# gift-surg/NSoL

Hardware: AMD Instinct MI355X
Metric: primal-dual iters/sec on 512^3 fp32 TV-L2 (higher is better)
Workload: dtype f32

## Files before the change

include/nsol_hip.h:

```cpp
#ifndef NSOL_HIP_H
#define NSOL_HIP_H

#include <stdint.h>

#ifdef __cplusplus
extern "C" {
#endif

#define NSOL_HIP_ABI_VERSION 1
#define NSOL_EINVAL (-1)

#define NSOL_MODE_CONSTANT 0
#define NSOL_MODE_WRAP 1
#define NSOL_MODE_NEAREST 2
#define NSOL_MODE_REFLECT 3
#define NSOL_MODE_MIRROR 4

#define NSOL_PD_REG_TV 0
#define NSOL_PD_REG_HUBER 1
#define NSOL_PD_DATA_L2 0
#define NSOL_PD_DATA_L1 2
#define NSOL_PD_REG_ISOTROPIC 4
#define NSOL_PD_DATA_WEIGHTED 8
#define NSOL_PD_RUN_X_MAY_SWAP 0x100
// ... 255 lines not shown
                            int64_t nx, double wx, double wy, double wz, int k,
                            const double *sigma_k, const double *hden_k,
                            const double *tau_k, const double *tl_k,
                            const double *theta_k, int flags, void *stream);
int nsol_pd_fusedk_tuned(int elem_size, int k, int64_t nz, int64_t ny, int64_t nx);
int nsol_pd_fusedk_launches(int k);
int nsol_pd_fusedk_tail2(int elem_size, int64_t nz, int64_t ny, int64_t nx);
int nsol_pd_fusedk_plan(int elem_size, int k, int64_t nz, int64_t ny, int64_t nx,
                        int *waves, int *ntx, int64_t *zchunk);
int nsol_pd_shift_launches(void);
int nsol_pd_shift_min_iters(int elem_size, int ndim, int64_t nz, int64_t ny, int64_t nx,
                            int flags, int64_t pitch);
int nsol_pd_fusedk_plan_form(int elem_size, int k, int64_t nz, int64_t ny, int64_t nx,
                             int form, int *waves, int *ntx, int64_t *zchunk);
int nsol_pd_run_parts(int iterations, int min_iters, int *lead, int *launches);
int64_t nsol_pd_persist_ws_bytes(int elem_size, int ndim, int64_t nz, int64_t ny,
                                 int64_t nx, int iterations);
int nsol_pd_persist_run_f32(float *xbar, float *x, const float *bt, float *p, int ndim,
                            int64_t nz, int64_t ny, int64_t nx, double wx, double wy,
                            double wz, double lambda, const double *sigma_host,
                            const double *tau_host, const double *theta_host,
                            int iterations, int p_is_zero, double gamma_huber, int flags,
                            void *ws, int64_t ws_bytes, unsigned int *err_word,
                            void *stream);
int nsol_pd_persist_run_f64(double *xbar, double *x, const double *bt, double *p, int ndim,
                            int64_t nz, int64_t ny, int64_t nx, double wx, double wy,
                            double wz, double lambda, const double *sigma_host,
                            const double *tau_host, const double *theta_host,
                            int iterations, int p_is_zero, double gamma_huber, int flags,
                            void *ws, int64_t ws_bytes, unsigned int *err_word,
// ... 578 lines not shown
```

nsol_amd/_lib.py:

```python
import ctypes
import os
import re

HERE = os.path.dirname(os.path.abspath(__file__))
LIB_PATH = os.path.join(HERE, "csrc", "libnsol_hip.so")
HEADER = os.path.join(HERE, "..", "include", "nsol_hip.h")

_lib = None

c_i64 = ctypes.c_int64
c_int = ctypes.c_int
c_dbl = ctypes.c_double
c_ptr = ctypes.c_void_p

_CTYPE = {"int": c_int, "int64_t": c_i64, "double": c_dbl}


class NsolHipError(RuntimeError):
    pass


def declared_symbols(header=HEADER):
    text = open(header).read()
    text = re.sub(r"/\*.*?\*/", "", text, flags=re.S)
# ... 64 lines not shown
    return lib


def check(rc, what):
    if rc != 0:
        if rc == -1:
            raise ValueError("%s: invalid argument" % what)
        raise NsolHipError("%s failed with hipError_t %d" % (what, rc))


PARAM_DEFAULTS = {
    "pd_zchunk": 0, "pd_ry": 0, "pd_two_pass": 0, "pd_xcd_map": 1, "pd_rag": 1,
    "max_grid_blocks": 2048, "stencil_slabs": 1, "stencil_blocks": 65536,
    "pd2_zchunk": 0, "pd2_enable": 1, "pd2_variant": 0, "pd2_xcd_map": 1,
    "pdk_enable": 1, "pdk_kmax": 3, "pdk_nw": 0, "pdk_zchunk": 0, "pdk_ntx": 0,
    "pdk_xcd_map": 1, "pdk_verbose": 0, "pdk_autotune": 1, "pdk_pf2": -1,
    "pdk_split": -1, "pdk_tail2": 1, "pdk_min_kvox": 1024, "pdk_tune_min_mvox": 16,
    "pdk_shift": -1, "pdk_shift_min_iters": 30,
    "pdp_max_spin": 1 << 21, "pdp_mute_tile": -1,
    "corr_ra": 8, "corr_xv": 1, "corr_blur3_lxb": 16, "corr_blur3_zchunk": 0, "corr_blur3_dma": 1, "corr_blur3_dma_rag": 1, "lb_gram_dma": 1, "lb_gram_mfma": 1, "sort_walk_by_key": 1,
}
_touched = set()


def reset_params():
    for name in sorted(_touched):
        set_param(name, PARAM_DEFAULTS[name])
    _touched.clear()


def set_param(name, value):
# ... 19 lines not shown
```

nsol_amd/csrc/nsol_pd_common.hpp:

```cpp
#pragma once

#include "nsol_common.hpp"

namespace nsol {

template <typename T, int V>
struct Pack {
  typedef T type __attribute__((ext_vector_type(V)));
};

template <typename T, int V>
__device__ __forceinline__ void ldv(const T *p, T (&v)[V]) {
  if constexpr (V == 1) {
    v[0] = *p;
  } else {
    typedef typename Pack<T, V>::type P;
    const P t = *reinterpret_cast<const P *>(p);
#pragma unroll
    for (int k = 0; k < V; ++k) v[k] = t[k];
  }
}

template <typename T, int V>
__device__ __forceinline__ void stv(T *p, const T (&v)[V]) {
// ... 114 lines not shown
                   const double *hden, const double *tau, const double *tl,
                   const double *theta, int flags, void *stream, int64_t pitch);

template <typename T>
int pd_shift3_min_iters(const T *x, const T *x_alt, const T *bt, const T *p0, const T *p1,
                        int ndim, int64_t nz, int64_t ny, int64_t nx, int flags,
                        int64_t pitch, int iterations);
template <typename T>
int pd_shift3_donation(int64_t nz, int64_t ny, int64_t nx);
template <typename T>
int pd_shift3_iter(const T *x_in, T *x_out, const T *bt, const T *p_in, T *p_out, int ndim,
                   int64_t nz, int64_t ny, int64_t nx, double wx, double wy, double wz,
                   const double *sigma, const double *hden, const double *tau,
                   const double *tl, const double *theta, int flags, void *stream);

template <bool L1, typename T>
__device__ __forceinline__ T prox_data_s(T u, T bt, T tl, T one_plus_tl) {
  if constexpr (L1) return prox_ell1(u, bt, tl);
  else return prox_ell2(u, bt, tl, one_plus_tl);
}

}
```

nsol_amd/csrc/nsol_pdk.hip:

```cpp
#include <stdio.h>
#include <string.h>

#include <algorithm>
#include <atomic>
#include <deque>
#include <map>
#include <mutex>
#include <tuple>
#include <type_traits>
#include <vector>

#include "nsol_common.hpp"
#include "nsol_pd_common.hpp"

using namespace nsol;

#ifndef PDK_LH
#define PDK_LH 1
#endif
#ifndef PDK_ABLATE
#define PDK_ABLATE 0
#endif
#ifndef PDK_PRIO
#define PDK_PRIO 0
#endif
#ifndef PDK_LOAD_AUX
#define PDK_LOAD_AUX 0
#endif

namespace nsol_pdk {

template <typename T, int K>
struct StageScalars {
  T sigma[K], hden[K], tau[K], tl[K], optl[K], theta[K];
  int has_p;
};

std::atomic<int> g_launches[2];
std::atomic<int> g_shift_launches;

struct Tiling {
  int lxb;
  int rows;
  int xv;
// ... 111 lines not shown
};

template <typename T, int V>
struct PlaneLoads {
  T xn[V], xv[V], btn[V], pxo[V], pyo[V], pzo[V], xdown[V], xup[V], pyup[V];
  T xright, xleft, pxleft;
};

template <typename T, int VEC, int NW, int K, int WPE, bool HUBER, bool L1, bool PF2,
          bool UNIT, bool RAG>
__global__ __launch_bounds__(NW * 64, WPE) void k_pd_fusedk(
    const T *__restrict__ xbar_in, T *__restrict__ xbar_out,
    const T *__restrict__ x_in, T *__restrict__ x_out,
    const T *__restrict__ bt, const T *__restrict__ p_in,
    T *__restrict__ p_out, Geom<T> G, StageScalars<T, K> S, Tiling Q, int zchunk,
    int slab) {
  constexpr int NT = NW * 64;
  constexpr int H = K - 1;
  constexpr int HX = ((H + VEC - 1) / VEC) * VEC;
  constexpr int LN = LdsShape<NT, K>::N;
  constexpr bool LH = PDK_LH && K == 3 && NW == 12 && !PF2 && sizeof(T) == 4 && !RAG;
  constexpr int NB = LH ? 1 : 2;
  __shared__ __attribute__((aligned(16))) T s_xb[NB][K - 1][LN * VEC];
  __shared__ __attribute__((aligned(16))) T s_py[NB][K - 1][LN * VEC];
  __shared__ T s_px[NB][K - 1][LN];
  __shared__ __attribute__((aligned(16))) T s_xb0[LH ? LN * VEC : VEC];
  __shared__ __attribute__((aligned(16))) T s_py0[LH ? LN * VEC : VEC];
  __shared__ T s_px0[LH ? LN : 1];

  const int tid = threadIdx.x;
  const int lane = tid & 63;
  const int ntiles = Q.ntx * Q.nty;
  int tile, zc;
  if (slab > 0) {
    const int xcd = blockIdx.x & 7;
    const int j = blockIdx.x >> 3;
    tile = xcd * slab + j % slab;
    zc = j / slab;
    if (tile >= ntiles) return;
  } else {
    tile = blockIdx.x % ntiles;
    zc = blockIdx.x / ntiles;
  }
  const int tx = tile % Q.ntx;
  const int ty = tile / Q.ntx;

  const int lxb = Q.lxb;
  constexpr int HL = HX / VEC;
  int row, lx;
  bool lone = false;
  if (Q.split) {
    const int inner = lxb - 2 * HL;
    const int main = Q.rows * inner;
    if (tid < main) {
      row = tid / inner;
      lx = HL + (tid - row * inner);
      lone = (lx == HL) || (lx == HL + inner - 1);
    } else {
// ... 479 lines not shown
  if constexpr (PF2) {
    for (; s + 1 <= s_hi; s += 2) {
      step(std::true_type{}, s, LA, LB, CA, CB);
      step(std::true_type{}, s + 1, LB, LA, CB, CA);
    }
    if (s <= s_hi) {
      step(std::true_type{}, s, LA, LB, CA, CB);
      CA = CB;
      ++s;
    }
  } else {
    for (; s <= s_hi; ++s) step(std::true_type{}, s, LA, LA, CA, CA);
  }
  for (; s <= s_last; ++s)
    step(std::false_type{}, s, LA, LA, CA, CA);
}

template <typename T>
struct ShiftScalars {
  T sigma[4], hden[4];
  T tau[3], tl[3], optl[3], theta[3];
};

template <typename T, int V>
struct ShiftLoads {
  T xv[V], btn[V], pxo[V], pyo[V], pzo[V], pyup[V];
  T pxleft;
};

template <typename T, int VEC, int NW, int WPE, bool HUBER, bool L1, bool PF2, bool UNIT>
__global__ __launch_bounds__(NW * 64, WPE) void k_pd_shift3(
    const T *__restrict__ x_in, T *__restrict__ x_out, const T *__restrict__ bt,
    const T *__restrict__ p_in, T *__restrict__ p_out, Geom<T> G, ShiftScalars<T> S,
    Tiling Q, int zchunk, int slab) {
  constexpr int K = 3;
  constexpr int NT = NW * 64;
  constexpr int HA = 2, HB = 3;
  constexpr int HX = ((K + VEC - 1) / VEC) * VEC;
  static_assert(HX >= K, "the x halo must hold the three voxels the right-hand cone needs");
  constexpr int LN = LdsShape<NT, K>::N;
  __shared__ __attribute__((aligned(16))) T s_xb[2][K][LN * VEC];
  __shared__ __attribute__((aligned(16))) T s_py[2][LN * VEC];
  __shared__ T s_px[2][LN];

  const int tid = threadIdx.x;
  const int lane = tid & 63;
  const int ntiles = Q.ntx * Q.nty;
  int tile, zc;
  if (slab > 0) {
    const int xcd = blockIdx.x & 7;
    const int j = blockIdx.x >> 3;
    tile = xcd * slab + j % slab;
    zc = j / slab;
    if (tile >= ntiles) return;
  } else {
    tile = blockIdx.x % ntiles;
    zc = blockIdx.x / ntiles;
  }
  const int tx = tile % Q.ntx;
  const int ty = tile / Q.ntx;

  const int lxb = Q.lxb;
  constexpr int HL = HX / VEC;
  int row, lx;
  bool lone = false;
  if (Q.split) {
    const int inner = lxb - 2 * HL;
    const int main = Q.rows * inner;
    if (tid < main) {
      row = tid / inner;
      lx = HL + (tid - row * inner);
      lone = (lx == HL) || (lx == HL + inner - 1);
    } else {
// ... 294 lines not shown
  if constexpr (PF2) {
    for (; s + 1 <= s_hi; s += 2) {
      step(std::true_type{}, s, LA, LB, CA, CB);
      step(std::true_type{}, s + 1, LB, LA, CB, CA);
    }
    if (s <= s_hi) {
      step(std::true_type{}, s, LA, LB, CA, CB);
      CA = CB;
      ++s;
    }
  } else {
    for (; s <= s_hi; ++s) step(std::true_type{}, s, LA, LA, CA, CA);
  }
  for (; s <= s_last; ++s)
    step(std::false_type{}, s, LA, LA, CA, CA);
}

struct Tuning {
  int enable = 1;
  int kmax = 3;
  int nw = 0;
  int zchunk = 0;
  int ntx = 0;
  int xcd_map = 1;
  int verbose = 0;
  int autotune = 1;
  int tune_min_mvox = 16;
  int pf2 = -1;
  int tail2 = 1;
  int min_kvox = 1024;
};
Tuning g_tunek;

int g_split = -1;

struct Config {
  int nw = 0;
  int pf2 = 0;
  Tiling q{};
  int64_t zchunk = 0;
  double cost = 0.0;
};

inline bool make_tiling(int64_t nx, int64_t ny, int nt, int vec, int h, int hx,
                        int lxm, int ntx, Tiling *out, int64_t xv_fixed = 0, int lost = -1) {
  if (lost < 0) lost = 2 * h;
  Tiling q;
  if (ntx == 1) {
    q.xv = 0;
    q.lxb = (int)((nx + vec - 1) / vec);
  } else {
    int64_t xv = xv_fixed > 0 ? xv_fixed : (nx + ntx - 1) / ntx;
    xv = (xv + vec - 1) / vec * vec;
    if (xv * (ntx - 1) >= nx) return false;
    q.xv = (int)xv;
    q.lxb = (int)(xv / vec) + 2 * (hx / vec);
  }
  if (q.lxb < 1 || q.lxb > lxm) return false;
  q.rows = nt / q.lxb;
  if (q.rows - lost < 1) return false;
  q.ntx = ntx;
  q.nty = (int)((ny + (q.rows - lost) - 1) / (q.rows - lost));
  q.split = (ntx > 1 && (q.xv / vec) % 32 == 0 && g_split != 0) ? 1 : 0;
  *out = q;
  return true;
}

inline double pick_zchunk(int64_t nz, int64_t tiles, int extra, int64_t max_chunk,
                          int64_t *chunk_out) {
  const double slots = (double)cu_count();
  double best = -1.0;
  int64_t best_chunk = nz < max_chunk ? nz : max_chunk;
  for (int64_t nzc = 1; nzc <= nz; ++nzc) {
    const int64_t chunk = (nz + nzc - 1) / nzc;
    if (chunk < 8 && nzc > 1) break;
    if (chunk > max_chunk) continue;
    if ((nz + chunk - 1) / chunk != nzc) continue;
    const double blocks = (double)tiles * nzc;
    const double rounds = (double)(int64_t)((blocks + slots - 1) / slots);
    const double fill = blocks / (rounds * slots);
// ... 3 lines not shown
  *chunk_out = best_chunk;
  return best > 0.0 ? best : 1.0;
}

inline double model_cost(const Tiling &q, int64_t nx, int64_t ny, int64_t nz,
                         int vec, int esize, int h, int hx, double zeff, bool shift = false) {
  double lines = 0.0;
  for (int tx = 0; tx < q.ntx; ++tx) {
    int64_t lo = q.xv ? (int64_t)tx * q.xv - hx : 0;
    int64_t hi = lo + (int64_t)q.lxb * vec;
    if (lo < 0) lo = 0;
    if (hi > nx) hi = nx;
    if (hi <= lo) continue;
    lines += (double)((hi * esize - 1) / 128 - (lo * esize) / 128 + 1);
  }
  double rows = 0.0;
  const int64_t tyv = q.rows - (shift ? 2 * h + 1 : 2 * h);
  for (int ty = 0; ty < q.nty; ++ty) {
    int64_t lo = (int64_t)ty * tyv - h, hi = lo + q.rows;
    if (lo < 0) lo = 0;
    if (hi > ny) hi = ny;
    if (hi > lo) rows += (double)(hi - lo);
  }
  const double reads = lines * 128.0 * rows * (double)nz * (shift ? 5.0 : 6.0);
  const double writes = (shift ? 4.0 : 5.0) * (double)nx * ny * nz * esize;
  return (reads + writes) / zeff;
}

template <typename T, int VEC, int NW, int K, int WPE, bool HUBER, bool L1, bool PF2,
          bool UNIT, bool RAG>
int launch_f(const Config &c, const T *xbar_in, T *xbar_out, const T *x_in, T *x_out,
             const T *bt, const T *p_in, T *p_out, const Geom<T> &G,
             const StageScalars<T, K> &S, hipStream_t st) {
  const Tiling &Q = c.q;
  const int64_t tiles = (int64_t)Q.ntx * Q.nty;
  const int64_t nzc = (G.nz + c.zchunk - 1) / c.zchunk;
  int64_t blocks = tiles * nzc;
  int64_t slab = 0;
  if (g_tunek.xcd_map && tiles >= 16) {
    slab = (tiles + 7) / 8;
    blocks = 8 * slab * nzc;
  }
  if (blocks > 0x7fffffff) return NSOL_EINVAL;
  if (g_tunek.verbose == 1)
    fprintf(stderr, "k_pd_fusedk K=%d waves=%d pf2=%d split=%d: lxb=%d rows=%d xv=%d tiles=%dx%d "
            "zchunk=%lld blocks=%lld slab=%lld model=%.3f GB\n", K, NW, (int)PF2, Q.split, Q.lxb, Q.rows,
            Q.xv, Q.ntx, Q.nty, (long long)c.zchunk, (long long)blocks,
            (long long)slab, c.cost * 1e-9);
  hipLaunchKernelGGL((k_pd_fusedk<T, VEC, NW, K, WPE, HUBER, L1, PF2, UNIT, RAG>),
                     dim3((unsigned)blocks), dim3(NW * 64), 0, st, xbar_in, xbar_out,
                     x_in, x_out, bt, p_in, p_out, G, S, Q, (int)c.zchunk, (int)slab);
  g_launches[K == 3 ? 1 : 0].fetch_add(1, std::memory_order_relaxed);
  return launch_status();
}

template <typename T, int VEC, int NW, int K, int WPE, bool PF2, bool RAG>
int launch_k(const Config &c, const T *xbar_in, T *xbar_out, const T *x_in, T *x_out,
             const T *bt, const T *p_in, T *p_out, const Geom<T> &G,
             const StageScalars<T, K> &S, int flags, hipStream_t st) {
#define NSOL_F(HB, L)                                                           \
  (unit ? launch_f<T, VEC, NW, K, WPE, HB, L, PF2, true, RAG>(                  \
              c, xbar_in, xbar_out, x_in, x_out, bt, p_in, p_out, G, S, st)     \
        : launch_f<T, VEC, NW, K, WPE, HB, L, PF2, false, RAG>(                 \
              c, xbar_in, xbar_out, x_in, x_out, bt, p_in, p_out, G, S, st))
  const bool unit = G.wx == T(1) && G.wy == T(1) && G.wz == T(1);
  const bool huber = (flags & NSOL_PD_REG_HUBER) != 0;
// ... 22 lines not shown
  }
  if (c.nw == 8) return c.pf2 ? NSOL_W(8, 2, true) : NSOL_W(8, 2, false);
  if constexpr (K == 2) {
    if (c.nw == 12) return NSOL_W(12, 3, false);
    if (c.nw == 16) return NSOL_W(16, 4, false);
  } else {
    if (c.nw == 12) return NSOL_W(12, 3, false);
  }
#undef NSOL_W
  return NSOL_EINVAL;
}

template <int NT, int K> constexpr int lxm_of() { return LdsShape<NT, K>::LXM; }

template <typename T, int K, bool SHIFT = false>
std::vector<Config> candidates(const Geom<T> &G) {
  constexpr int VW = 16 / sizeof(T);
  constexpr int H = K - 1;
  constexpr int HX = (((SHIFT ? K : H) + VW - 1) / VW) * VW;
  constexpr int LOST = SHIFT ? 2 * H + 1 : 2 * H;
  std::vector<Config> out;
  const int64_t plane_bytes = G.sz * (int64_t)sizeof(T);
  const int64_t max_planes = ((int64_t)1 << 30) / plane_bytes - 1;
  const int64_t max_chunk = max_planes - 2 * K - 1;
  if (max_chunk < 8) return out;
  for (int wi = 0; wi < Waves<K>::n; ++wi) {
    const int nw = Waves<K>::v[wi];
    if (g_tunek.nw > 0 && g_tunek.nw != nw) continue;
    if (G.nx % VW != 0 && nw != 12) continue;
    if (SHIFT && g_tunek.pf2 == 0 && nw == 8) continue;
    const int nt = nw * 64;
// ... 1 lines not shown
    struct Spec { int ntx; int64_t xv; };
    std::vector<Spec> specs;
    for (int ntx = 1; ntx <= 64; ++ntx) specs.push_back({ntx, 0});
    for (int lanes : {64, 128}) {
      const int64_t xv = (int64_t)lanes * VW;
      if (G.nx > xv && G.nx % xv != 0)
        specs.push_back({(int)((G.nx + xv - 1) / xv), xv});
    }
    for (const Spec &sp : specs) {
      const int ntx = sp.ntx;
      if (g_tunek.ntx > 0 && ntx != g_tunek.ntx) continue;
      Config c;
      c.nw = nw;
      c.pf2 = (nw == 8) ? 1 : 0;
      if (g_tunek.pf2 == 0) c.pf2 = 0;
      if (!make_tiling(G.nx, G.ny, nt, VW, H, HX, lxm, ntx, &c.q, sp.xv, LOST)) continue;
      const int64_t tiles = (int64_t)c.q.ntx * c.q.nty;
      double zeff;
      if (g_tunek.zchunk > 0) {
        c.zchunk = g_tunek.zchunk < max_chunk ? g_tunek.zchunk : max_chunk;
        if (c.zchunk > G.nz) c.zchunk = G.nz;
        zeff = (double)c.zchunk / (double)(c.zchunk + LOST);
      } else {
        zeff = pick_zchunk(G.nz, tiles, LOST, max_chunk, &c.zchunk);
      }
      c.cost = model_cost(c.q, G.nx, G.ny, G.nz, VW, (int)sizeof(T), H, HX, zeff, SHIFT);
      c.cost *= 1.0 + 0.02 * (16 - nw) / 4.0;
      if (c.q.split) {
        const bool whole = ((c.q.lxb - 2 * (HX / VW)) % 64) == 0;
        if (!whole) {
          Config d = c;
          d.q.split = 0;
          out.push_back(d);
        }
        c.cost *= whole ? 0.88 : 0.97;
      }
      out.push_back(c);
    }
  }
  std::sort(out.begin(), out.end(),
            [](const Config &a, const Config &b) { return a.cost < b.cost; });
  return out;
}

struct PlanKey {
  int device, esize, k;
  int64_t nz, ny, nx;
  int64_t pitch = 0;
  int form = 0;
  bool operator<(const PlanKey &o) const {
    return std::tie(device, esize, k, nz, ny, nx, pitch, form) <
           std::tie(o.device, o.esize, o.k, o.nz, o.ny, o.nx, o.pitch, o.form);
// ... 59 lines not shown
    if (P.done[i] < plan_target(P, i, best_now)) all = false;
  if (all) {
    auto score = [&](int i) {
      if ((int)P.samples[i].size() < kFinalRounds) return P.best_ms[i] * kFinalBand;
      std::vector<float> v(P.samples[i].begin() + 1, P.samples[i].end());
      std::sort(v.begin(), v.end());
      return v[1];
    };
    int arg = 0;
    for (int i = 0; i < n; ++i)
      if (!P.dropped[i] && (P.dropped[arg] || score(i) < score(arg))) arg = i;
    P.chosen = arg;
    if (g_tunek.verbose) {
      for (int i = 0; i < n; ++i)
      {
        fprintf(stderr, "k_pd_fusedk tune K=%d waves=%d ntx=%d zchunk=%lld: %.3f ms%s  [",
                K, P.cand[i].nw, P.cand[i].q.ntx, (long long)P.cand[i].zchunk,
                P.best_ms[i], i == arg ? "  <- kept" : (P.dropped[i] ? "  (dropped)" : ""));
        for (float v : P.samples[i]) fprintf(stderr, " %.3f", v);
        fprintf(stderr, " ]\n");
      }
    }
  }
}

template <typename T, int K, bool SHIFT, typename Go>
int planned_launch(const Geom<T> &G, bool sample, hipStream_t st, Go go);

inline std::vector<Config> short_list(const std::vector<Config> &cand) {
  std::vector<Config> out;
  int per_nw[17] = {0};
  for (const Config &c : cand)
    if (per_nw[c.nw]++ < 1 || c.q.ntx <= 4) out.push_back(c);
  return out;
}

template <typename T, int K>
int fusedk_k(const T *xbar_in, T *xbar_out, const T *x_in, T *x_out, const T *bt,
             const T *p_in, T *p_out, const Geom<T> &G, const double *sigma,
             const double *hden, const double *tau, const double *tl,
             const double *theta, int flags, hipStream_t st) {
  StageScalars<T, K> S;
  for (int i = 0; i < K; ++i) {
    S.sigma[i] = (T)sigma[i]; S.hden[i] = huber_den<T>(hden[i]); S.tau[i] = (T)tau[i];
    S.tl[i] = (T)tl[i]; S.optl[i] = prox_den<T>(tl[i]); S.theta[i] = (T)theta[i];
  }
  S.has_p = p_in != nullptr ? 1 : 0;
  return planned_launch<T, K, false>(G, S.has_p != 0, st, [&](const Config &cfg) {
    return launch_cfg<T, K>(cfg, xbar_in, xbar_out, x_in, x_out, bt, p_in, p_out, G, S,
                            flags, st);
  });
}

template <typename T, int K, bool SHIFT, typename Go>
int planned_launch(const Geom<T> &G, bool sample, hipStream_t st, Go go) {
#define NSOL_GO(cfg) go(cfg)
  const bool forced = g_tunek.nw > 0 || g_tunek.ntx > 0 || g_tunek.zchunk > 0;
  if (forced) {
    std::vector<Config> cand = candidates<T, K, SHIFT>(G);
    if (cand.empty()) return -2;
    return NSOL_GO(cand[0]);
  }
  const PlanKey key{current_device(), (int)sizeof(T), K, G.nz, G.ny, G.nx,
                    G.padded ? G.sy : 0, SHIFT ? 1 : 0};
  std::lock_guard<std::mutex> lock(g_plans_mutex);
  auto it = g_plans.find(key);
  if (it == g_plans.end()) {
    Plan P;
    std::vector<Config> cand = candidates<T, K, SHIFT>(G);
    if (cand.empty()) return -2;
    const bool big = G.n >= ((int64_t)g_tunek.tune_min_mvox << 20);
    int seeded = -1;
    if (K == 2 && g_tunek.autotune && big) {
      auto it3 = g_plans.find(PlanKey{key.device, key.esize, 3, G.nz, G.ny, G.nx, key.pitch});
      if (it3 == g_plans.end() || it3->second.chosen < 0)
        it3 = g_plans.find(PlanKey{key.device, key.esize, 3, G.nz, G.ny, G.nx, key.pitch, 1});
      if (it3 != g_plans.end() && it3->second.chosen >= 0) {
        const Config &c3 = it3->second.cand[it3->second.chosen];
        for (int i = 0; i < (int)cand.size() && seeded < 0; ++i)
          if (cand[i].nw == 12 && cand[i].q.ntx == 1) seeded = i;
        for (int i = 0; i < (int)cand.size() && seeded < 0; ++i)
          if (cand[i].nw == c3.nw && cand[i].q.ntx == c3.q.ntx) seeded = i;
      }
    }
    bool shortlist = false;
    if (K == 3 && !SHIFT && g_tunek.autotune && big) {
      auto its = g_plans.find(PlanKey{key.device, key.esize, 3, G.nz, G.ny, G.nx, key.pitch, 1});
      shortlist = its != g_plans.end();
    }
    if (seeded >= 0) {
      P.cand.push_back(cand[seeded]);
      P.chosen = 0;
    } else if (shortlist && cand.size() > 1) {
      P.cand = short_list(cand);
    } else if (SHIFT && g_tunek.autotune && big && cand.size() > 1) {
      int per_nw[17] = {0};
      for (const Config &c : cand) {
        const int rank = per_nw[c.nw]++;
        if (rank >= 3 && c.q.ntx > 4) continue;
        P.cand.push_back(c);
        const int64_t zc = c.zchunk > 96 ? 64 : 24;
        if (rank < 2 && zc < c.zchunk && zc <= G.nz) {
          Config d = c;
          d.zchunk = zc;
          P.cand.push_back(d);
        }
      }
    } else if (g_tunek.autotune && big && cand.size() > 1) {
      int per_nw[17] = {0};
      for (const Config &c : cand) {
        if (per_nw[c.nw]++ >= 5 && c.q.ntx > 8) continue;
        P.cand.push_back(c);
        const int64_t zc = c.zchunk > 96 ? 64 : 24;
        if (zc < c.zchunk && zc <= G.nz) {
          Config d = c;
          d.zchunk = zc;
          P.cand.push_back(d);
        }
      }
    } else {
      P.cand.push_back(cand[0]);
      P.chosen = 0;
    }
    const size_t n = P.cand.size();
    P.best_ms.assign(n, -1.f);
    P.samples.assign(n, std::vector<float>());
// ... 51 lines not shown
int g_shift = -1;
int g_shift_min_iters = 30;

inline int shift_threshold() {
  if (g_shift > 0) return 4;
  return g_shift_min_iters > 4 ? g_shift_min_iters : 4;
}

template <typename T, int VEC, int NW, int WPE, bool PF2>
int launch_shift(const Config &c, const T *x_in, T *x_out, const T *bt, const T *p_in,
                 T *p_out, const Geom<T> &G, const ShiftScalars<T> &S, int flags,
                 hipStream_t st) {
  const Tiling &Q = c.q;
  const int64_t tiles = (int64_t)Q.ntx * Q.nty;
  const int64_t nzc = (G.nz + c.zchunk - 1) / c.zchunk;
  int64_t blocks = tiles * nzc;
  int64_t slab = 0;
  if (g_tunek.xcd_map && tiles >= 16) {
    slab = (tiles + 7) / 8;
    blocks = 8 * slab * nzc;
  }
  if (blocks > 0x7fffffff) return NSOL_EINVAL;
  if (g_tunek.verbose == 1)
    fprintf(stderr, "k_pd_shift3 waves=%d pf2=%d split=%d: lxb=%d rows=%d xv=%d tiles=%dx%d "
            "zchunk=%lld blocks=%lld slab=%lld model=%.3f GB\n", NW, (int)PF2, Q.split, Q.lxb,
            Q.rows, Q.xv, Q.ntx, Q.nty, (long long)c.zchunk, (long long)blocks,
            (long long)slab, c.cost * 1e-9);
#define NSOL_S(HB, L, U)                                                             \
  hipLaunchKernelGGL((k_pd_shift3<T, VEC, NW, WPE, HB, L, PF2, U>), dim3((unsigned)blocks), \
                     dim3(NW * 64), 0, st, x_in, x_out, bt, p_in, p_out, G, S, Q,    \
                     (int)c.zchunk, (int)slab)
#define NSOL_SU(HB, L) do { if (unit) NSOL_S(HB, L, true); else NSOL_S(HB, L, false); } while (0)
  const bool unit = G.wx == T(1) && G.wy == T(1) && G.wz == T(1);
  const bool huber = (flags & NSOL_PD_REG_HUBER) != 0;
  const bool l1 = (flags & NSOL_PD_DATA_L1) != 0;
  if (huber) { if (l1) NSOL_SU(true, true); else NSOL_SU(true, false); }
  else { if (l1) NSOL_SU(false, true); else NSOL_SU(false, false); }
#undef NSOL_SU
#undef NSOL_S
  g_launches[1].fetch_add(1, std::memory_order_relaxed);
  g_shift_launches.fetch_add(1, std::memory_order_relaxed);
  return launch_status();
}

template <typename T>
int shift_donation(const Geom<T> &G) {
  if (!g_tunek.autotune || G.n < ((int64_t)g_tunek.tune_min_mvox << 20) || g_tunek.nw > 0 ||
      g_tunek.ntx > 0 || g_tunek.zchunk > 0)
    return -1;
  std::lock_guard<std::mutex> lock(g_plans_mutex);
  const int dev = current_device();
  auto its = g_plans.find(PlanKey{dev, (int)sizeof(T), 3, G.nz, G.ny, G.nx, 0, 1});
  if (its == g_plans.end()) return 0;
  plan_poll(its->second, 3);
  if (its->second.chosen < 0) {
    const Plan &S = its->second;
    const float sbest = plan_best(S);
    for (int i = 0; i < (int)S.cand.size(); ++i)
      if (S.issued[i] < plan_target(S, i, sbest)) return 0;
  }
  auto it = g_plans.find(PlanKey{dev, (int)sizeof(T), 3, G.nz, G.ny, G.nx, 0, 0});
  if (it == g_plans.end()) {
    const std::vector<Config> cand = candidates<T, 3, false>(G);
    if (cand.size() < 2) return -1;
    return (int)short_list(cand).size() * kFinalRounds + 1;
  }
  Plan &P = it->second;
  plan_poll(P, 3);
  if (P.chosen >= 0) return -1;
  const float best = plan_best(P);
  int want = 0;
  for (int i = 0; i < (int)P.cand.size(); ++i) {
    const int owed = plan_target(P, i, best) - P.issued[i];
    if (owed > 0) want += owed;
  }
  return want + 1;
}

// ... 5 lines not shown
  if (n < ((int64_t)g_tunek.min_kvox << 10) || nx % VW != 0 || nx / VW < 8 || ny < 8 ||
      nz < 8 || nz >= ((int64_t)1 << 30))
    return false;
  return g_shift > 0 || n >= ((int64_t)g_tunek.tune_min_mvox << 20);
}
inline bool shift_shape_ok(int elem_size, int64_t nz, int64_t ny, int64_t nx) {
  return elem_size == 4 ? shift_shape_ok<float>(3, nz, ny, nx, 0)
                        : shift_shape_ok<double>(3, nz, ny, nx, 0);
}

template <typename T>
int shift_min_iters_t(int ndim, int64_t nz, int64_t ny, int64_t nx, int64_t pitch) {
  if (!shift_shape_ok<T>(ndim, nz, ny, nx, pitch)) return 0;
  const Geom<T> G = make_geom<T>(ndim, nz, ny, nx, 1.0, 1.0, 1.0);
  std::lock_guard<std::mutex> lock(g_plans_mutex);
  const bool forced = g_tunek.nw > 0 || g_tunek.ntx > 0 || g_tunek.zchunk > 0;
  if (forced || g_plans.find(PlanKey{current_device(), (int)sizeof(T), 3, nz, ny, nx, 0,
                                     1}) == g_plans.end())
    if (candidates<T, 3, true>(G).empty()) return 0;
  return shift_threshold();
}

}

namespace nsol {

template <typename T>
int pd_shift3_min_iters(const T *x, const T *x_alt, const T *bt, const T *p0, const T *p1,
                        int ndim, int64_t nz, int64_t ny, int64_t nx, int flags,
                        int64_t pitch, int iterations) {
  if (!nsol_pdk::g_shift || iterations < nsol_pdk::shift_threshold()) return 0;
// ... 94 lines not shown
NSOL_PDK_INST(double)
#undef NSOL_PDK_INST

}

extern "C" {

int nsol_hip_set_param_pdk(const char *name, int value) {
  if (!name) return NSOL_EINVAL;
  if (!strcmp(name, "pdk_enable")) nsol_pdk::g_tunek.enable = value;
  else if (!strcmp(name, "pdk_kmax")) nsol_pdk::g_tunek.kmax = value;
  else if (!strcmp(name, "pdk_nw")) nsol_pdk::g_tunek.nw = value;
  else if (!strcmp(name, "pdk_zchunk")) nsol_pdk::g_tunek.zchunk = value;
  else if (!strcmp(name, "pdk_ntx")) nsol_pdk::g_tunek.ntx = value;
  else if (!strcmp(name, "pdk_xcd_map")) nsol_pdk::g_tunek.xcd_map = value;
  else if (!strcmp(name, "pdk_verbose")) nsol_pdk::g_tunek.verbose = value;
  else if (!strcmp(name, "pdk_autotune")) nsol_pdk::g_tunek.autotune = value;
  else if (!strcmp(name, "pdk_pf2")) nsol_pdk::g_tunek.pf2 = value;
  else if (!strcmp(name, "pdk_split")) nsol_pdk::g_split = value;
  else if (!strcmp(name, "pdk_min_kvox")) nsol_pdk::g_tunek.min_kvox = value;
  else if (!strcmp(name, "pdk_tail2")) nsol_pdk::g_tunek.tail2 = value;
  else if (!strcmp(name, "pdk_tune_min_mvox")) nsol_pdk::g_tunek.tune_min_mvox = value;
  else if (!strcmp(name, "pdk_shift")) nsol_pdk::g_shift = value < 0 ? -1 : (value ? 1 : 0);
  else if (!strcmp(name, "pdk_shift_min_iters")) nsol_pdk::g_shift_min_iters = value;
  else if (!strcmp(name, "pdk_forget")) {
    std::lock_guard<std::mutex> lock(nsol_pdk::g_plans_mutex);
    for (auto &kv : nsol_pdk::g_plans)
      for (auto &sm : kv.second.pending) {
        (void)hipEventDestroy(sm.e0);
        (void)hipEventDestroy(sm.e1);
// ... 94 lines not shown
int nsol_pd_fusedk_plan(int elem_size, int k, int64_t nz, int64_t ny, int64_t nx,
                        int *waves, int *ntx, int64_t *zchunk) {
  std::lock_guard<std::mutex> lock(nsol_pdk::g_plans_mutex);
  const int form = (k == 3 && nsol_pdk::shift_shape_ok(elem_size, nz, ny, nx)) ? 1 : 0;
  auto it = nsol_pdk::g_plans.find(
      nsol_pdk::PlanKey{nsol_pdk::current_device(), elem_size, k, nz, ny, nx, 0, form});
  if (form && it == nsol_pdk::g_plans.end())
    it = nsol_pdk::g_plans.find(
        nsol_pdk::PlanKey{nsol_pdk::current_device(), elem_size, k, nz, ny, nx, 0, 0});
  if (it == nsol_pdk::g_plans.end() || it->second.chosen < 0) return NSOL_EINVAL;
  const nsol_pdk::Config &c = it->second.cand[it->second.chosen];
  if (waves) *waves = c.nw;
  if (ntx) *ntx = c.q.ntx;
  if (zchunk) *zchunk = c.zchunk;
  return 0;
}

#define NSOL_PDK_DEF(T, SUF)                                                           \
  int nsol_pd_fusedk_iter_pitched_##SUF(                                               \
      const T *xbar_in, T *xbar_out, const T *x_in, T *x_out, const T *bt, const T *p_in, \
      T *p_out, int ndim, int64_t nz, int64_t ny, int64_t nx, int64_t pitch, double wx, \
      double wy, double wz, int k, const double *sigma, const double *hden,            \
      const double *tau, const double *tl, const double *theta, int flags,             \
      void *stream) {                                                                  \
    return pd_fusedk_iter<T>(xbar_in, xbar_out, x_in, x_out, bt, p_in, p_out, ndim,    \
                             nz, ny, nx, wx, wy, wz, k, sigma, hden, tau, tl, theta,   \
                             flags, stream, pitch);                                    \
  }                                                                                    \
  int nsol_pd_fusedk_iter_##SUF(                                                       \
      const T *xbar_in, T *xbar_out, const T *x_in, T *x_out, const T *bt, const T *p_in, \
// ... 13 lines not shown
```

Measured before the change: 3064.

## Map contiguous tile-row bands to each XCD and autotune trimmed row heights

New measurement: 3133, median of 6. 2.2% higher.

```diff
diff --git a/include/nsol_hip.h b/include/nsol_hip.h
--- a/include/nsol_hip.h
+++ b/include/nsol_hip.h
@@ -293,6 +293,8 @@
 int nsol_pd_fusedk_plan_form(int elem_size, int k, int64_t nz, int64_t ny, int64_t nx,
                              int form, int *waves, int *ntx, int64_t *zchunk);
 int nsol_pd_run_parts(int iterations, int min_iters, int *lead, int *launches);
+int nsol_pdk_block_map(int mode, int ntx, int nty, int nzc, int *out, int max_blocks);
+int nsol_pdk_finish_probe(int64_t *out, int words);
 int64_t nsol_pd_persist_ws_bytes(int elem_size, int ndim, int64_t nz, int64_t ny,
                                  int64_t nx, int iterations);
 int nsol_pd_persist_run_f32(float *xbar, float *x, const float *bt, float *p, int ndim,
diff --git a/nsol_amd/_lib.py b/nsol_amd/_lib.py
--- a/nsol_amd/_lib.py
+++ b/nsol_amd/_lib.py
@@ -102,7 +102,7 @@
     "max_grid_blocks": 2048, "stencil_slabs": 1, "stencil_blocks": 65536,
     "pd2_zchunk": 0, "pd2_enable": 1, "pd2_variant": 0, "pd2_xcd_map": 1,
     "pdk_enable": 1, "pdk_kmax": 3, "pdk_nw": 0, "pdk_zchunk": 0, "pdk_ntx": 0,
-    "pdk_xcd_map": 1, "pdk_verbose": 0, "pdk_autotune": 1, "pdk_pf2": -1,
+    "pdk_xcd_map": 1, "pdk_rows": 0, "pdk_verbose": 0, "pdk_autotune": 1, "pdk_pf2": -1,
     "pdk_split": -1, "pdk_tail2": 1, "pdk_min_kvox": 1024, "pdk_tune_min_mvox": 16,
     "pdk_shift": -1, "pdk_shift_min_iters": 30,
     "pdp_max_spin": 1 << 21, "pdp_mute_tile": -1,
diff --git a/nsol_amd/csrc/nsol_pd_common.hpp b/nsol_amd/csrc/nsol_pd_common.hpp
--- a/nsol_amd/csrc/nsol_pd_common.hpp
+++ b/nsol_amd/csrc/nsol_pd_common.hpp
@@ -152,6 +152,59 @@
                    const double *sigma, const double *hden, const double *tau,
                    const double *tl, const double *theta, int flags, void *stream);
 
+struct PdkBlockMap {
+  int mode;
+  int ntx, nty;
+  int nzc;
+  int q;
+  int big;
+};
+__host__ __device__ inline PdkBlockMap pdk_block_map(int want, int ntx, int nty, int nzc) {
+  PdkBlockMap M{0, ntx, nty, nzc, 0, 8};
+  if (want == 1 && nty >= 8) {
+    M.mode = 1;
+    M.q = nty / 8;
+    M.big = 8 - nty % 8;
+  } else if (want == 2 && ntx * nty >= 16) {
+    M.mode = 2;
+    M.q = (ntx * nty + 7) / 8;
+  }
+  return M;
+}
+__host__ __device__ inline long long pdk_map_blocks(const PdkBlockMap &M) {
+  if (M.mode == 1) return 8LL * (M.q + (M.big < 8 ? 1 : 0)) * M.ntx * M.nzc;
+  if (M.mode == 2) return 8LL * M.q * M.nzc;
+  return (long long)M.ntx * M.nty * M.nzc;
+}
+__host__ __device__ inline void pdk_map_xcd_rows(const PdkBlockMap &M, int x, int &first,
+                                                 int &count) {
+  const int over = x > M.big ? x - M.big : 0;
+  first = x * M.q + over;
+  count = M.q + (x >= M.big ? 1 : 0);
+}
+__host__ __device__ inline bool pdk_block_tile(const PdkBlockMap &M, int b, int &tile,
+                                               int &zc) {
+  const int ntiles = M.ntx * M.nty;
+  if (M.mode == 1) {
+    int first, count;
+    pdk_map_xcd_rows(M, b & 7, first, count);
+    const int j = b >> 3;
+    const int per = count * M.ntx;
+    zc = j / per;
+    tile = first * M.ntx + (j - zc * per);
+    return zc < M.nzc;
+  }
+  if (M.mode == 2) {
+    const int j = b >> 3;
+    tile = (b & 7) * M.q + j % M.q;
+    zc = j / M.q;
+    return tile < ntiles;
+  }
+  tile = b % ntiles;
+  zc = b / ntiles;
+  return true;
+}
+
 template <bool L1, typename T>
 __device__ __forceinline__ T prox_data_s(T u, T bt, T tl, T one_plus_tl) {
   if constexpr (L1) return prox_ell1(u, bt, tl);
diff --git a/nsol_amd/csrc/nsol_pdk.hip b/nsol_amd/csrc/nsol_pdk.hip
--- a/nsol_amd/csrc/nsol_pdk.hip
+++ b/nsol_amd/csrc/nsol_pdk.hip
@@ -28,6 +28,18 @@
 #define PDK_LOAD_AUX 0
 #endif
 
+#ifdef NSOL_PDK_FINISH_PROBE
+constexpr int kProbeBlocks = 8192;
+__device__ unsigned long long g_finish_probe[2 * kProbeBlocks];
+#define PDK_PROBE_MARK(w)                                                      \
+  do {                                                                         \
+    if (threadIdx.x == 0 && blockIdx.x < (unsigned)kProbeBlocks)               \
+      g_finish_probe[2 * blockIdx.x + (w)] = wall_clock64();                   \
+  } while (0)
+#else
+#define PDK_PROBE_MARK(w) do { } while (0)
+#endif
+
 namespace nsol_pdk {
 
 template <typename T, int K>
@@ -169,7 +181,7 @@
     const T *__restrict__ x_in, T *__restrict__ x_out,
     const T *__restrict__ bt, const T *__restrict__ p_in,
     T *__restrict__ p_out, Geom<T> G, StageScalars<T, K> S, Tiling Q, int zchunk,
-    int slab) {
+    PdkBlockMap M) {
   constexpr int NT = NW * 64;
   constexpr int H = K - 1;
   constexpr int HX = ((H + VEC - 1) / VEC) * VEC;
@@ -185,18 +197,9 @@
 
   const int tid = threadIdx.x;
   const int lane = tid & 63;
-  const int ntiles = Q.ntx * Q.nty;
   int tile, zc;
-  if (slab > 0) {
-    const int xcd = blockIdx.x & 7;
-    const int j = blockIdx.x >> 3;
-    tile = xcd * slab + j % slab;
-    zc = j / slab;
-    if (tile >= ntiles) return;
-  } else {
-    tile = blockIdx.x % ntiles;
-    zc = blockIdx.x / ntiles;
-  }
+  if (!pdk_block_tile(M, (int)blockIdx.x, tile, zc)) return;
+  PDK_PROBE_MARK(0);
   const int tx = tile % Q.ntx;
   const int ty = tile / Q.ntx;
 
@@ -706,6 +709,7 @@
   }
   for (; s <= s_last; ++s)
     step(std::false_type{}, s, LA, LA, CA, CA);
+  PDK_PROBE_MARK(1);
 }
 
 template <typename T>
@@ -724,7 +728,7 @@
 __global__ __launch_bounds__(NW * 64, WPE) void k_pd_shift3(
     const T *__restrict__ x_in, T *__restrict__ x_out, const T *__restrict__ bt,
     const T *__restrict__ p_in, T *__restrict__ p_out, Geom<T> G, ShiftScalars<T> S,
-    Tiling Q, int zchunk, int slab) {
+    Tiling Q, int zchunk, PdkBlockMap M) {
   constexpr int K = 3;
   constexpr int NT = NW * 64;
   constexpr int HA = 2, HB = 3;
@@ -737,18 +741,9 @@
 
   const int tid = threadIdx.x;
   const int lane = tid & 63;
-  const int ntiles = Q.ntx * Q.nty;
   int tile, zc;
-  if (slab > 0) {
-    const int xcd = blockIdx.x & 7;
-    const int j = blockIdx.x >> 3;
-    tile = xcd * slab + j % slab;
-    zc = j / slab;
-    if (tile >= ntiles) return;
-  } else {
-    tile = blockIdx.x % ntiles;
-    zc = blockIdx.x / ntiles;
-  }
+  if (!pdk_block_tile(M, (int)blockIdx.x, tile, zc)) return;
+  PDK_PROBE_MARK(0);
   const int tx = tile % Q.ntx;
   const int ty = tile / Q.ntx;
 
@@ -1073,6 +1068,7 @@
   }
   for (; s <= s_last; ++s)
     step(std::false_type{}, s, LA, LA, CA, CA);
+  PDK_PROBE_MARK(1);
 }
 
 struct Tuning {
@@ -1082,6 +1078,7 @@
   int zchunk = 0;
   int ntx = 0;
   int xcd_map = 1;
+  int rows = 0;
   int verbose = 0;
   int autotune = 1;
   int tune_min_mvox = 16;
@@ -1090,19 +1087,24 @@
   int min_kvox = 1024;
 };
 Tuning g_tunek;
+inline bool geometry_forced() {
+  return g_tunek.nw > 0 || g_tunek.ntx > 0 || g_tunek.zchunk > 0 || g_tunek.rows > 0;
+}
 
 int g_split = -1;
 
 struct Config {
   int nw = 0;
   int pf2 = 0;
+  int trimmed = 0;
   Tiling q{};
   int64_t zchunk = 0;
   double cost = 0.0;
 };
 
 inline bool make_tiling(int64_t nx, int64_t ny, int nt, int vec, int h, int hx,
-                        int lxm, int ntx, Tiling *out, int64_t xv_fixed = 0, int lost = -1) {
+                        int lxm, int ntx, Tiling *out, int64_t xv_fixed = 0, int lost = -1,
+                        int rows = 0) {
   if (lost < 0) lost = 2 * h;
   Tiling q;
   if (ntx == 1) {
@@ -1117,12 +1119,18 @@
   }
   if (q.lxb < 1 || q.lxb > lxm) return false;
   q.rows = nt / q.lxb;
+  if (rows > q.rows) return false;
+  if (rows > 0) q.rows = rows;
   if (q.rows - lost < 1) return false;
   q.ntx = ntx;
   q.nty = (int)((ny + (q.rows - lost) - 1) / (q.rows - lost));
   q.split = (ntx > 1 && (q.xv / vec) % 32 == 0 && g_split != 0) ? 1 : 0;
   *out = q;
   return true;
+}
+
+inline PdkBlockMap launch_map(const Tiling &q, int64_t nzc, bool ) {
+  return pdk_block_map(g_tunek.xcd_map, q.ntx, q.nty, (int)nzc);
 }
 
 inline double pick_zchunk(int64_t nz, int64_t tiles, int extra, int64_t max_chunk,
@@ -1156,13 +1164,27 @@
     if (hi <= lo) continue;
     lines += (double)((hi * esize - 1) / 128 - (lo * esize) / 128 + 1);
   }
-  double rows = 0.0;
   const int64_t tyv = q.rows - (shift ? 2 * h + 1 : 2 * h);
-  for (int ty = 0; ty < q.nty; ++ty) {
-    int64_t lo = (int64_t)ty * tyv - h, hi = lo + q.rows;
-    if (lo < 0) lo = 0;
-    if (hi > ny) hi = ny;
-    if (hi > lo) rows += (double)(hi - lo);
+  auto rows_of = [&](int ty0, int ty1) {
+    double r = 0.0;
+    for (int ty = ty0; ty < ty1; ++ty) {
+      int64_t lo = (int64_t)ty * tyv - h, hi = lo + q.rows;
+      if (lo < 0) lo = 0;
+      if (hi > ny) hi = ny;
+      if (hi > lo) r += (double)(hi - lo);
+    }
+    return r;
+  };
+  double rows = rows_of(0, q.nty);
+  const PdkBlockMap M = launch_map(q, 1, shift);
+  if (M.mode == 1) {
+    double heavy = 0.0;
+    for (int x = 0; x < 8; ++x) {
+      int first, count;
+      pdk_map_xcd_rows(M, x, first, count);
+      heavy = std::max(heavy, rows_of(first, first + count));
+    }
+    rows = 8.0 * heavy;
   }
   const double reads = lines * 128.0 * rows * (double)nz * (shift ? 5.0 : 6.0);
   const double writes = (shift ? 4.0 : 5.0) * (double)nx * ny * nz * esize;
@@ -1177,21 +1199,18 @@
   const Tiling &Q = c.q;
   const int64_t tiles = (int64_t)Q.ntx * Q.nty;
   const int64_t nzc = (G.nz + c.zchunk - 1) / c.zchunk;
-  int64_t blocks = tiles * nzc;
-  int64_t slab = 0;
-  if (g_tunek.xcd_map && tiles >= 16) {
-    slab = (tiles + 7) / 8;
-    blocks = 8 * slab * nzc;
-  }
+  if (tiles * nzc > 0x3fffffff) return NSOL_EINVAL;
+  const PdkBlockMap M = launch_map(Q, nzc, false);
+  const int64_t blocks = pdk_map_blocks(M);
   if (blocks > 0x7fffffff) return NSOL_EINVAL;
   if (g_tunek.verbose == 1)
     fprintf(stderr, "k_pd_fusedk K=%d waves=%d pf2=%d split=%d: lxb=%d rows=%d xv=%d tiles=%dx%d "
-            "zchunk=%lld blocks=%lld slab=%lld model=%.3f GB\n", K, NW, (int)PF2, Q.split, Q.lxb, Q.rows,
+            "zchunk=%lld blocks=%lld map=%d:%d model=%.3f GB\n", K, NW, (int)PF2, Q.split, Q.lxb, Q.rows,
             Q.xv, Q.ntx, Q.nty, (long long)c.zchunk, (long long)blocks,
-            (long long)slab, c.cost * 1e-9);
+            M.mode, M.q, c.cost * 1e-9);
   hipLaunchKernelGGL((k_pd_fusedk<T, VEC, NW, K, WPE, HUBER, L1, PF2, UNIT, RAG>),
                      dim3((unsigned)blocks), dim3(NW * 64), 0, st, xbar_in, xbar_out,
-                     x_in, x_out, bt, p_in, p_out, G, S, Q, (int)c.zchunk, (int)slab);
+                     x_in, x_out, bt, p_in, p_out, G, S, Q, (int)c.zchunk, M);
   g_launches[K == 3 ? 1 : 0].fetch_add(1, std::memory_order_relaxed);
   return launch_status();
 }
@@ -1244,7 +1263,7 @@
 template <int NT, int K> constexpr int lxm_of() { return LdsShape<NT, K>::LXM; }
 
 template <typename T, int K, bool SHIFT = false>
-std::vector<Config> candidates(const Geom<T> &G) {
+std::vector<Config> candidates(const Geom<T> &G, bool twins = false) {
   constexpr int VW = 16 / sizeof(T);
   constexpr int H = K - 1;
   constexpr int HX = (((SHIFT ? K : H) + VW - 1) / VW) * VW;
@@ -1276,28 +1295,54 @@
       c.nw = nw;
       c.pf2 = (nw == 8) ? 1 : 0;
       if (g_tunek.pf2 == 0) c.pf2 = 0;
-      if (!make_tiling(G.nx, G.ny, nt, VW, H, HX, lxm, ntx, &c.q, sp.xv, LOST)) continue;
-      const int64_t tiles = (int64_t)c.q.ntx * c.q.nty;
-      double zeff;
-      if (g_tunek.zchunk > 0) {
-        c.zchunk = g_tunek.zchunk < max_chunk ? g_tunek.zchunk : max_chunk;
-        if (c.zchunk > G.nz) c.zchunk = G.nz;
-        zeff = (double)c.zchunk / (double)(c.zchunk + LOST);
-      } else {
-        zeff = pick_zchunk(G.nz, tiles, LOST, max_chunk, &c.zchunk);
-      }
-      c.cost = model_cost(c.q, G.nx, G.ny, G.nz, VW, (int)sizeof(T), H, HX, zeff, SHIFT);
-      c.cost *= 1.0 + 0.02 * (16 - nw) / 4.0;
-      if (c.q.split) {
-        const bool whole = ((c.q.lxb - 2 * (HX / VW)) % 64) == 0;
-        if (!whole) {
+      if (!make_tiling(G.nx, G.ny, nt, VW, H, HX, lxm, ntx, &c.q, sp.xv, LOST, g_tunek.rows))
+        continue;
+      auto price = [&](Config &c) {
+        const int64_t tiles = (int64_t)c.q.ntx * c.q.nty;
+        double zeff;
+        if (g_tunek.zchunk > 0) {
+          c.zchunk = g_tunek.zchunk < max_chunk ? g_tunek.zchunk : max_chunk;
+          if (c.zchunk > G.nz) c.zchunk = G.nz;
+          zeff = (double)c.zchunk / (double)(c.zchunk + LOST);
+        } else {
+          zeff = pick_zchunk(G.nz, tiles, LOST, max_chunk, &c.zchunk);
+        }
+        c.cost = model_cost(c.q, G.nx, G.ny, G.nz, VW, (int)sizeof(T), H, HX, zeff, SHIFT);
+        c.cost *= 1.0 + 0.02 * (16 - nw) / 4.0;
+      };
+      auto push = [&](Config c) {
+        if (c.q.split) {
+          const bool whole = ((c.q.lxb - 2 * (HX / VW)) % 64) == 0;
+          if (!whole) {
+            Config d = c;
+            d.q.split = 0;
+            out.push_back(d);
+          }
+          c.cost *= whole ? 0.88 : 0.97;
+        }
+        out.push_back(c);
+      };
+      price(c);
+      push(c);
+      if (twins && g_tunek.rows == 0) {
+        auto nty_of = [&](int r) { return (int64_t)((G.ny + (r - LOST) - 1) / (r - LOST)); };
+        const int rmax = c.q.rows;
+        int twin[2] = {0, 0};
+        for (int r = rmax - 1; r >= rmax - 3 && r > LOST && !twin[0]; --r)
+          if (nty_of(r) % 8 == 0) twin[0] = r;
+        const int64_t waste = (int64_t)c.q.nty * (rmax - LOST) - G.ny;
+        for (int r = rmax - 1; r > LOST && !twin[1]; --r)
+          if (nty_of(r) * (r - LOST) - G.ny < waste) twin[1] = r;
+        if (twin[1] == twin[0]) twin[1] = 0;
+        for (int r : twin) {
           Config d = c;
-          d.q.split = 0;
-          out.push_back(d);
+          if (!r || !make_tiling(G.nx, G.ny, nt, VW, H, HX, lxm, ntx, &d.q, sp.xv, LOST, r))
+            continue;
+          d.trimmed = 1;
+          price(d);
+          if (d.cost < c.cost) push(d);
         }
-        c.cost *= whole ? 0.88 : 0.97;
-      }
-      out.push_back(c);
+      }
     }
   }
   std::sort(out.begin(), out.end(),
@@ -1387,8 +1432,8 @@
     if (g_tunek.verbose) {
       for (int i = 0; i < n; ++i)
       {
-        fprintf(stderr, "k_pd_fusedk tune K=%d waves=%d ntx=%d zchunk=%lld: %.3f ms%s  [",
-                K, P.cand[i].nw, P.cand[i].q.ntx, (long long)P.cand[i].zchunk,
+        fprintf(stderr, "k_pd_fusedk tune K=%d waves=%d ntx=%d zchunk=%lld rows=%d: %.3f ms%s  [",
+                K, P.cand[i].nw, P.cand[i].q.ntx, (long long)P.cand[i].zchunk, P.cand[i].q.rows,
                 P.best_ms[i], i == arg ? "  <- kept" : (P.dropped[i] ? "  (dropped)" : ""));
         for (float v : P.samples[i]) fprintf(stderr, " %.3f", v);
         fprintf(stderr, " ]\n");
@@ -1404,7 +1449,7 @@
   std::vector<Config> out;
   int per_nw[17] = {0};
   for (const Config &c : cand)
-    if (per_nw[c.nw]++ < 1 || c.q.ntx <= 4) out.push_back(c);
+    if (per_nw[c.nw]++ < 1 || (c.q.ntx <= 4 && !c.trimmed)) out.push_back(c);
   return out;
 }
 
@@ -1428,7 +1473,7 @@
 template <typename T, int K, bool SHIFT, typename Go>
 int planned_launch(const Geom<T> &G, bool sample, hipStream_t st, Go go) {
 #define NSOL_GO(cfg) go(cfg)
-  const bool forced = g_tunek.nw > 0 || g_tunek.ntx > 0 || g_tunek.zchunk > 0;
+  const bool forced = geometry_forced();
   if (forced) {
     std::vector<Config> cand = candidates<T, K, SHIFT>(G);
     if (cand.empty()) return -2;
@@ -1440,9 +1485,9 @@
   auto it = g_plans.find(key);
   if (it == g_plans.end()) {
     Plan P;
-    std::vector<Config> cand = candidates<T, K, SHIFT>(G);
+    const bool big = G.n >= ((int64_t)g_tunek.tune_min_mvox << 20);
+    std::vector<Config> cand = candidates<T, K, SHIFT>(G, K == 3 && g_tunek.autotune && big);
     if (cand.empty()) return -2;
-    const bool big = G.n >= ((int64_t)g_tunek.tune_min_mvox << 20);
     int seeded = -1;
     if (K == 2 && g_tunek.autotune && big) {
       auto it3 = g_plans.find(PlanKey{key.device, key.esize, 3, G.nz, G.ny, G.nx, key.pitch});
@@ -1470,7 +1515,7 @@
       int per_nw[17] = {0};
       for (const Config &c : cand) {
         const int rank = per_nw[c.nw]++;
-        if (rank >= 3 && c.q.ntx > 4) continue;
+        if (rank >= 3 && (c.q.ntx > 4 || c.trimmed)) continue;
         P.cand.push_back(c);
         const int64_t zc = c.zchunk > 96 ? 64 : 24;
         if (rank < 2 && zc < c.zchunk && zc <= G.nz) {
@@ -1482,7 +1527,7 @@
     } else if (g_tunek.autotune && big && cand.size() > 1) {
       int per_nw[17] = {0};
       for (const Config &c : cand) {
-        if (per_nw[c.nw]++ >= 5 && c.q.ntx > 8) continue;
+        if (per_nw[c.nw]++ >= 5 && (c.q.ntx > 8 || c.trimmed)) continue;
         P.cand.push_back(c);
         const int64_t zc = c.zchunk > 96 ? 64 : 24;
         if (zc < c.zchunk && zc <= G.nz) {
@@ -1564,22 +1609,19 @@
   const Tiling &Q = c.q;
   const int64_t tiles = (int64_t)Q.ntx * Q.nty;
   const int64_t nzc = (G.nz + c.zchunk - 1) / c.zchunk;
-  int64_t blocks = tiles * nzc;
-  int64_t slab = 0;
-  if (g_tunek.xcd_map && tiles >= 16) {
-    slab = (tiles + 7) / 8;
-    blocks = 8 * slab * nzc;
-  }
+  if (tiles * nzc > 0x3fffffff) return NSOL_EINVAL;
+  const PdkBlockMap M = launch_map(Q, nzc, true);
+  const int64_t blocks = pdk_map_blocks(M);
   if (blocks > 0x7fffffff) return NSOL_EINVAL;
   if (g_tunek.verbose == 1)
     fprintf(stderr, "k_pd_shift3 waves=%d pf2=%d split=%d: lxb=%d rows=%d xv=%d tiles=%dx%d "
-            "zchunk=%lld blocks=%lld slab=%lld model=%.3f GB\n", NW, (int)PF2, Q.split, Q.lxb,
+            "zchunk=%lld blocks=%lld map=%d:%d model=%.3f GB\n", NW, (int)PF2, Q.split, Q.lxb,
             Q.rows, Q.xv, Q.ntx, Q.nty, (long long)c.zchunk, (long long)blocks,
-            (long long)slab, c.cost * 1e-9);
+            M.mode, M.q, c.cost * 1e-9);
 #define NSOL_S(HB, L, U)                                                             \
   hipLaunchKernelGGL((k_pd_shift3<T, VEC, NW, WPE, HB, L, PF2, U>), dim3((unsigned)blocks), \
                      dim3(NW * 64), 0, st, x_in, x_out, bt, p_in, p_out, G, S, Q,    \
-                     (int)c.zchunk, (int)slab)
+                     (int)c.zchunk, M)
 #define NSOL_SU(HB, L) do { if (unit) NSOL_S(HB, L, true); else NSOL_S(HB, L, false); } while (0)
   const bool unit = G.wx == T(1) && G.wy == T(1) && G.wz == T(1);
   const bool huber = (flags & NSOL_PD_REG_HUBER) != 0;
@@ -1595,8 +1637,7 @@
 
 template <typename T>
 int shift_donation(const Geom<T> &G) {
-  if (!g_tunek.autotune || G.n < ((int64_t)g_tunek.tune_min_mvox << 20) || g_tunek.nw > 0 ||
-      g_tunek.ntx > 0 || g_tunek.zchunk > 0)
+  if (!g_tunek.autotune || G.n < ((int64_t)g_tunek.tune_min_mvox << 20) || geometry_forced())
     return -1;
   std::lock_guard<std::mutex> lock(g_plans_mutex);
   const int dev = current_device();
@@ -1611,7 +1652,7 @@
   }
   auto it = g_plans.find(PlanKey{dev, (int)sizeof(T), 3, G.nz, G.ny, G.nx, 0, 0});
   if (it == g_plans.end()) {
-    const std::vector<Config> cand = candidates<T, 3, false>(G);
+    const std::vector<Config> cand = candidates<T, 3, false>(G, true);
     if (cand.size() < 2) return -1;
     return (int)short_list(cand).size() * kFinalRounds + 1;
   }
@@ -1647,7 +1688,7 @@
   if (!shift_shape_ok<T>(ndim, nz, ny, nx, pitch)) return 0;
   const Geom<T> G = make_geom<T>(ndim, nz, ny, nx, 1.0, 1.0, 1.0);
   std::lock_guard<std::mutex> lock(g_plans_mutex);
-  const bool forced = g_tunek.nw > 0 || g_tunek.ntx > 0 || g_tunek.zchunk > 0;
+  const bool forced = geometry_forced();
   if (forced || g_plans.find(PlanKey{current_device(), (int)sizeof(T), 3, nz, ny, nx, 0,
                                      1}) == g_plans.end())
     if (candidates<T, 3, true>(G).empty()) return 0;
@@ -1772,6 +1813,7 @@
   else if (!strcmp(name, "pdk_zchunk")) nsol_pdk::g_tunek.zchunk = value;
   else if (!strcmp(name, "pdk_ntx")) nsol_pdk::g_tunek.ntx = value;
   else if (!strcmp(name, "pdk_xcd_map")) nsol_pdk::g_tunek.xcd_map = value;
+  else if (!strcmp(name, "pdk_rows")) nsol_pdk::g_tunek.rows = value;
   else if (!strcmp(name, "pdk_verbose")) nsol_pdk::g_tunek.verbose = value;
   else if (!strcmp(name, "pdk_autotune")) nsol_pdk::g_tunek.autotune = value;
   else if (!strcmp(name, "pdk_pf2")) nsol_pdk::g_tunek.pf2 = value;
@@ -1896,6 +1938,39 @@
   if (ntx) *ntx = c.q.ntx;
   if (zchunk) *zchunk = c.zchunk;
   return 0;
+}
+
+int nsol_pdk_block_map(int mode, int ntx, int nty, int nzc, int *out, int max_blocks) {
+  if (mode < 0 || mode > 2 || ntx < 1 || nty < 1 || nzc < 1 || !out ||
+      (int64_t)ntx * nty * nzc > 0x3fffffff)
+    return NSOL_EINVAL;
+  const nsol::PdkBlockMap M = nsol::pdk_block_map(mode, ntx, nty, nzc);
+  const long long blocks = nsol::pdk_map_blocks(M);
+  if (blocks > max_blocks) return NSOL_EINVAL;
+  for (int b = 0; b < (int)blocks; ++b) {
+    int tile, zc;
+    const bool live = nsol::pdk_block_tile(M, b, tile, zc);
+    out[2 * b] = live ? tile : -1;
+    out[2 * b + 1] = live ? zc : -1;
+  }
+  return (int)blocks;
+}
+
+int nsol_pdk_finish_probe(int64_t *out, int words) {
+#ifdef NSOL_PDK_FINISH_PROBE
+  if (!out || words < 0 || words > 2 * kProbeBlocks) return NSOL_EINVAL;
+  if (hipDeviceSynchronize() != hipSuccess) return launch_status();
+  if (hipMemcpyFromSymbol(out, HIP_SYMBOL(g_finish_probe), (size_t)words * 8) != hipSuccess)
+    return launch_status();
+  void *table = nullptr;
+  if (hipGetSymbolAddress(&table, HIP_SYMBOL(g_finish_probe)) != hipSuccess ||
+      hipMemset(table, 0, sizeof(unsigned long long) * 2 * kProbeBlocks) != hipSuccess)
+    return launch_status();
+  return 0;
+#else
+  (void)out; (void)words;
+  return -2;
+#endif
 }
 
 #define NSOL_PDK_DEF(T, SUF)                                                           \
```
